# Qixiaomao/video-caption-algorithm

Hardware: AMD Instinct MI355X
Metric: captions/sec + p50 encode+decode latency, 16-frame ViT-B/16 → GPT-2-small, 1/2/4/8 GPU (higher is better)
Workload: dtype bf16

## Files before the change

include/vcap.h:

```cpp
#ifndef VCAP_H_
#define VCAP_H_

#include <stddef.h>
#include <stdint.h>

#ifdef __cplusplus
extern "C" {
#endif

#define VCAP_ABI_VERSION 16

enum { VCAP_DT_F32 = 0, VCAP_DT_BF16 = 1, VCAP_DT_MXFP8 = 2, VCAP_DT_F16 = 3 };
enum { VCAP_E_ARG = -1000, VCAP_E_WORKSPACE = -1001, VCAP_E_UNSUPPORTED = -1002 };

typedef struct vcap_vit_layer {
  const float* ln1_g; const float* ln1_b;
  const void* qkv_w; const float* qkv_b;
  const void* proj_w; const float* proj_b;
  const float* ln2_g; const float* ln2_b;
  const void* fc1_w; const float* fc1_b;
  const void* fc2_w; const float* fc2_b;
  const uint8_t* qkv_ws; const uint8_t* proj_ws; const uint8_t* fc1_ws; const uint8_t* fc2_ws;
} vcap_vit_layer;

// ... 88 lines not shown
                           size_t ws_bytes, void* stream);

size_t vcap_mx_scale_bytes(int rows, int K);
int vcap_vit_attention_mx(const void* qkv, void* out, uint8_t* out_scales, int frames, int tokens, int heads,
                          void* stream);
int vcap_mx_quantize(int in_dtype, const void* x, int64_t ldx, int rows, int K, void* q, uint8_t* scales,
                     void* stream);
int vcap_layernorm_mx(const float* x, int64_t ldx, void* q, uint8_t* scales, const float* gamma, const float* beta,
                      int rows, int dim, float eps, void* stream);
int vcap_gemm_mx(const void* A, const uint8_t* a_scales, const void* W, const uint8_t* w_scales, int out_dtype,
                 void* C, int64_t ldc, uint8_t* c_scales, int M, int N, int K, const float* bias, int act,
                 const float* res, void* stream);
int vcap_vit_pool_temporal(int dtype, const void* feat, void* out, int bsz, int timesteps, int tokens, int channels,
                           int pool_gap, void* stream);
int vcap_prefix_project(const float* emb, int B, int video_dim, const vcap_prefix_desc* pd, float* prefix_out,
                        void* stream);

size_t vcap_rows_packed_bytes(int dtype, int N, int K);
int vcap_rows_pack(int dtype, const void* w, int64_t ldw, int N, int K, void* packed, void* stream);

size_t vcap_vit_workspace_bytes(const vcap_vit_desc* d, int B, int T);
int vcap_vit_encode(const vcap_vit_desc* d, const vcap_prefix_desc* pd, const float* frames, int B, int T,
                    float* enc_out, float* prefix_out, void* workspace, size_t ws_bytes, void* stream);
int vcap_vit_layer_fuses_qkv_attention(const vcap_vit_desc* d, int layer);

size_t vcap_gpt2_workspace_bytes(const vcap_gpt2_desc* d, int B, int S0, int max_new_tokens);
int vcap_gpt2_generate(const vcap_gpt2_desc* d, const vcap_gen_params* gp, const float* prefix, const int* prompt_ids,
                       int prompt_len, int B, int* out_ids, float* logits_out, void* workspace, size_t ws_bytes,
                       void* stream);
typedef struct vcap_sample_params {
  float temperature;
  int top_k;
  double top_p;
  uint64_t seed;
} vcap_sample_params;
int vcap_gpt2_sample(const vcap_gpt2_desc* d, const vcap_gen_params* gp, const vcap_sample_params* sp,
                     const float* prefix, const int* prompt_ids, int prompt_len, int B, int* out_ids,
                     float* logits_out, float* warped_out, const int* force_ids, void* workspace, size_t ws_bytes,
                     void* stream);
void vcap_graph_cache_clear(void);
int vcap_graph_cache_size(void);
int vcap_gpt2_max_rows(void);

int vcap_decode_attention(int dtype, const void* q, const void* k_pool, const void* v_pool, const int* page_table,
                          int maxp, void* out, int M, int heads, int S_new, int past, void* stream);

// ... 156 lines not shown
```

video-caption-algorithm_amd/csrc/gemm256.hip:

```cpp
#include <cstdlib>

#include "vcap_common.h"
#include "vcap_kernels.h"

namespace {

constexpr int TM = 256, TN = 256, ROWB = 128;
constexpr int HALF = 128 * ROWB;
constexpr int BUF = 4 * HALF;
constexpr int LDS_BYTES = 2 * BUF;
constexpr int SBUF = 2048;
constexpr int LDS_BYTES_MX = LDS_BYTES + 4 * SBUF;

VCAP_DEV void glds16(const void* g, char* lds_wave_base) {
  __builtin_amdgcn_global_load_lds((const __attribute__((address_space(1))) void*)g,
                                   (__attribute__((address_space(3))) void*)lds_wave_base, 16, 0, 0);
}

template <typename T, int GS>
VCAP_DEV void half_offsets(uint32_t (&off)[2], long ld, int rows, int base, int X, int wave, int lane) {
  constexpr int E = Frag<T>::kElems;
#pragma unroll
  for (int i = 0; i < 2; ++i) {
    const int lr = (wave * 2 + i) * 8 + (lane >> 3);
// ... 139 lines not shown
          r[i][j] = *reinterpret_cast<const f32x4*>(epi.res + (long)m * epi.ldr + n);
        }
    };
    auto res_store = [&](const f32x4 (&r)[4][2], int qm, int qn) {
#pragma unroll
      for (int i = 0; i < 4; ++i)
#pragma unroll
        for (int j = 0; j < 2; ++j) {
          const int m = m0 + wr * 128 + qm * 64 + i * 16 + fr;
          const int n = n0 + wc * 64 + qn * 32 + j * 16 + fg * 4;
          const f32x4 v = Autocast<TIn>::rnd4(acc[qm][qn][i][j] + bias[qn][j]) + r[i][j];
          if (m < M && n < N) out_store(reinterpret_cast<f32x4*>(C + (long)m * ldc + n), v);
        }
    };
    f32x4 r0[4][2], r1[4][2];
    res_load(r0, 0, 0);
    res_load(r1, 0, 1);
    res_store(r0, 0, 0);
    res_load(r0, 1, 0);
    res_store(r1, 0, 1);
    res_load(r1, 1, 1);
    res_store(r0, 1, 0);
    res_store(r1, 1, 1);
  } else {
#pragma unroll
  for (int qm = 0; qm < 2; ++qm)
#pragma unroll
    for (int qn = 0; qn < 2; ++qn)
#pragma unroll
      for (int j = 0; j < 2; ++j) {
        const int n = n0 + wc * 64 + qn * 32 + j * 16 + fg * 4;
        if (n >= N) continue;
        const f32x4 bias = epi.bias ? *reinterpret_cast<const f32x4*>(epi.bias + n) : (f32x4){0.f, 0.f, 0.f, 0.f};
#pragma unroll
        for (int i = 0; i < 4; ++i) {
          const int m = m0 + wr * 128 + qm * 64 + i * 16 + fr;
          if (m >= M) continue;
          f32x4 v = acc[qm][qn][i][j] + bias;
          if constexpr (!(EPI == 0 && sizeof(TOut) == 2)) v = Autocast<TIn>::rnd4(v);
          long orow = m;
          if constexpr (EPI == 1) {
#pragma unroll
            for (int e = 0; e < 4; ++e) v[e] = gelu_tanh(v[e]);
          } else if constexpr (EPI == 2) {
            v += *reinterpret_cast<const f32x4*>(epi.res + orow * epi.ldr + n);
          } else if constexpr (EPI == 3) {
// ... 258 lines not shown
    if (w > 0 && w < tiles_n && tiles_n % w == 0) e.colgroup = w;
  }
  hipLaunchKernelGGL((vcap_gemm256_kernel<TIn, TOut, EPI>), dim3(tiles), dim3(512), lds, s, (const TIn*)A, lda,
                     (const TIn*)W, ldw, (TOut*)C, ldc, M, N, K, e);
  return hipGetLastError();
}

template <typename TIn, typename TOut>
static hipError_t launch256(const void* A, long lda, const void* W, long ldw, void* C, long ldc, int M, int N, int K,
                            const GemmEpi& epi, hipStream_t s) {
  if constexpr (sizeof(TOut) == 1) {
    return launch256_epi<TIn, TOut, 4>(A, lda, W, ldw, C, ldc, M, N, K, epi, s);
  } else {
    const bool plain_rows = epi.G == 0;
    if (plain_rows && epi.res_mode == 0 && epi.act == 0)
      return launch256_epi<TIn, TOut, 0>(A, lda, W, ldw, C, ldc, M, N, K, epi, s);
    if constexpr (sizeof(TOut) == sizeof(TIn) || sizeof(TOut) == 2) {
      if (plain_rows && epi.res_mode == 0 && epi.act == 1)
        return launch256_epi<TIn, TOut, 1>(A, lda, W, ldw, C, ldc, M, N, K, epi, s);
    }
    if constexpr (sizeof(TOut) == 4) {
      if (plain_rows && epi.res_mode == 1 && epi.act == 0 && epi.res == (const float*)C && epi.ldr == ldc)
        return launch256_epi<TIn, TOut, 2>(A, lda, W, ldw, C, ldc, M, N, K, epi, s);
    }
    return launch256_epi<TIn, TOut, 3>(A, lda, W, ldw, C, ldc, M, N, K, epi, s);
  }
}

bool vcap_gemm256_ok(int in_dt, int out_dt, long lda, long ldw, long ldc, int M, int N, int K, const GemmEpi& epi) {
  if (!vcap_dt_size(in_dt) || !vcap_dt_size(out_dt)) return false;
  const int bk = 128 / (int)vcap_dt_size(in_dt);
  if (K % (2 * bk) != 0 || N % 16 != 0 || M <= 0) return false;
  const int ein = 16 / (int)vcap_dt_size(in_dt);
  if (in_dt == VCAP_DT_MXFP8 && (!epi.a_scale || !epi.w_scale)) return false;
  if (out_dt == VCAP_DT_MXFP8 && (in_dt != VCAP_DT_MXFP8 || N % 128 || ldc % 16 || epi.act != 1 || !epi.bias ||
                                  !epi.c_scale || epi.G || epi.res_mode))
    return false;
  if (lda % ein || ldw % ein) return false;
  if (ldc % 4) return false;
  if (epi.bias && ((uintptr_t)epi.bias & 15)) return false;
  if (epi.res && (((uintptr_t)epi.res & 15) || epi.ldr % 4)) return false;
  (void)out_dt;
  return true;
}

hipError_t vcap_gemm256_dispatch(int in_dt, int out_dt, const void* A, long lda, const void* W, long ldw, void* C,
// ... 20 lines not shown
```

video-caption-algorithm_amd/csrc/runtime_vit.hip:

```cpp
#include "runtime_common.h"

namespace {

struct VitBufs {
  float* x;
  void* xn;
  void* qkv;
  void* attn;
  void* act;
  uint8_t* xn_s;
  uint8_t* act_s;
  float* splitk;
  size_t splitk_bytes;
};

int vit_adt(int dt) { return dt == VCAP_DT_MXFP8 ? VCAP_DT_BF16 : dt; }

VitBufs carve_vit(Carver& c, const vcap_vit_desc* d, int B, int T) {
  const int tokens = (d->image / d->patch) * (d->image / d->patch) + 1;
  const size_t M = (size_t)B * T * tokens;
  const size_t es = esize(d->dtype), ea = esize(vit_adt(d->dtype));
  const size_t npatch = (size_t)B * T * (tokens - 1);
  VitBufs v;
  const size_t en = es > ea ? es : ea;
// ... 24 lines not shown
    return fail(VCAP_E_UNSUPPORTED, "vit dims must be multiples of the GEMM K step");
  if (d->dtype == VCAP_DT_MXFP8) {
    if (d->dim > 1024) return fail(VCAP_E_UNSUPPORTED, "MXFP8 LayerNorm holds rows of <= 1024 in registers");
    if (d->dim % 256 || d->mlp % 256) return fail(VCAP_E_UNSUPPORTED, "MXFP8 dims must be multiples of 256");
  }
  if (d->image % d->patch) return fail(VCAP_E_ARG, "image not divisible by patch");
  const int tokens = (d->image / d->patch) * (d->image / d->patch) + 1;
  if (tokens > 288) return fail(VCAP_E_UNSUPPORTED, "more than 288 tokens");
  if (!vcap_vit_attention_supported(vit_adt(d->dtype), tokens))
    return fail(VCAP_E_UNSUPPORTED, "vit attention serves 33..192 and 225..256 tokens in fp16 only");
  if (!vcap_vit_head_prefix_supported(d->dim, 1)) return fail(VCAP_E_UNSUPPORTED, "vit dim > 1024 (the head holds a row in LDS)");
  if (!vcap_vit_head_prefix_supported(1, d->video_dim)) return fail(VCAP_E_UNSUPPORTED, "video_dim > 1024");
  return 0;
}

bool vit_layer_fused(const vcap_vit_desc* d, const vcap_vit_layer& ly) {
  const bool mx = d->dtype == VCAP_DT_MXFP8;
  const int g = d->image / d->patch;
  return !(mx && ly.qkv_ws) && !(mx && ly.proj_ws) && vcap_vit_qkv_attention_supported(vit_adt(d->dtype), g * g + 1, d->heads);
}

std::string vit_site(const char* name, bool last) { return std::string("vit.") + name + (last ? ".cls" : ""); }

}

extern "C" {

int vcap_vit_attention(int dtype, const void* qkv, void* out, int frames, int tokens, int heads, void* stream) {
  if (!qkv || !out || frames <= 0 || tokens <= 0 || heads <= 0) return fail(VCAP_E_ARG, "vcap_vit_attention: bad arguments");
  if (tokens > 288) return fail(VCAP_E_UNSUPPORTED, "vcap_vit_attention: tokens > 288");
  VCAP_TRY(vcap_vit_attention_dispatch(dtype, qkv, out, frames, tokens, heads, (hipStream_t)stream),
           "vcap_vit_attention");
  return 0;
}

int vcap_vit_qkv_attention_dt(int dtype, const void* xn, const void* wqkv, const float* bqkv, void* out, int frames,
                              int tokens, int heads, int cls_only, void* stream) {
  if (!xn || !wqkv || !bqkv || !out || frames <= 0 || tokens <= 0 || heads <= 0)
    return fail(VCAP_E_ARG, "vcap_vit_qkv_attention: bad arguments");
  if (dtype != VCAP_DT_BF16 && dtype != VCAP_DT_F16)
    return fail(VCAP_E_ARG, "vcap_vit_qkv_attention: dtype must be VCAP_DT_BF16 or VCAP_DT_F16");
  if (!vcap_vit_qkv_attention_supported(dtype, tokens, heads))
    return fail(VCAP_E_UNSUPPORTED, "vcap_vit_qkv_attention: needs 192 < tokens <= 208 (ViT-B/16) or 256 < tokens <= 272 (ViT-L/14) "
                "and heads*64 <= 4096");
  VCAP_TRY(vcap_vit_qkv_attention_dispatch(dtype, xn, wqkv, bqkv, out, frames, tokens, heads, cls_only ? 1 : 0,
                                           (hipStream_t)stream),
// ... 33 lines not shown
                        void* stream) {
  if (!emb || !pd || !prefix_out || !pd->mapper_w || B <= 0) return fail(VCAP_E_ARG, "vcap_prefix_project: bad arguments");
  if (!vcap_vit_head_prefix_supported(1, video_dim)) return fail(VCAP_E_UNSUPPORTED, "video_dim > 1024");
  VCAP_TRY(vcap_vit_head_prefix_dispatch(nullptr, B, 1, 1, 1, nullptr, nullptr, 0.f, nullptr, nullptr, video_dim,
                                         pd->ln_scale, pd->in_weight, pd->mapper_w, pd->mapper_b,
                                         pd->prefix_len * pd->n_embd, nullptr, prefix_out, emb, nullptr,
                                         (hipStream_t)stream),
           "vcap_prefix_project");
  return 0;
}

size_t vcap_vit_workspace_bytes(const vcap_vit_desc* d, int B, int T) {
  return check_vit(d) ? 0 : carved_bytes([&](Carver& c) { carve_vit(c, d, B, T); });
}

int vcap_vit_layer_fuses_qkv_attention(const vcap_vit_desc* d, int layer) {
  if (int rc = check_vit(d)) return rc;
  if (layer < 0 || layer >= d->depth) return fail(VCAP_E_ARG, "vcap_vit_layer_fuses_qkv_attention: layer out of range");
  return vit_layer_fused(d, d->layers[layer]) ? 1 : 0;
}

int vcap_vit_encode(const vcap_vit_desc* d, const vcap_prefix_desc* pd, const float* frames, int B, int T,
                    float* enc_out, float* prefix_out, void* workspace, size_t ws_bytes, void* stream) {
  if (int rc = check_vit(d)) return rc;
  if (!frames || !enc_out || B <= 0 || T <= 0) return fail(VCAP_E_ARG, "vcap_vit_encode: bad arguments");
  if (prefix_out && (!pd || !pd->mapper_w)) return fail(VCAP_E_ARG, "vcap_vit_encode: prefix desc missing");
  if (ws_bytes < vcap_vit_workspace_bytes(d, B, T)) return fail(VCAP_E_WORKSPACE, "vcap_vit_encode: workspace too small");
  hipStream_t s = (hipStream_t)stream;
  Carver c(workspace);
  VitBufs w = carve_vit(c, d, B, T);
  const int dt = d->dtype, D = d->dim, g = d->image / d->patch, P = g * g, N = P + 1, BT = B * T;
  const int adt = vit_adt(dt);
  const bool mx = dt == VCAP_DT_MXFP8;
  const int M = BT * N;
  auto norm = [&](bool mxq, long ldx, const float* gamma, const float* beta, int rows, const char* where) -> int {
    if (mxq)
      VCAP_TRY(vcap_layernorm_mx_dispatch(w.x, ldx, (uint8_t*)w.xn, w.xn_s, rows, gamma, beta, rows, D, d->ln_eps, s),
               where);
    else
      VCAP_TRY(vcap_layernorm_dispatch(adt, w.x, ldx, w.xn, D, gamma, beta, rows, D, d->ln_eps, s), where);
    return 0;
  };
  VCAP_TRY(vcap_patchify_dispatch(adt, frames, w.act, w.x, d->cls, d->pos, BT, d->image, d->patch, d->kpad, N, D, s),
           "patchify");
  GemmEpi pe{d->patch_b, d->pos, D, 0, 2, P, N, 1, 1};
  VCAP_TRY(vcap_gemm_dispatch(adt, VCAP_DT_F32, w.act, d->kpad, d->patch_w, d->kpad, w.x, D, BT * P, D, d->kpad, pe, s),
           "patch_gemm");
  for (int l = 0; l < d->depth; ++l) {
    const vcap_vit_layer& ly = d->layers[l];
    const bool last = l == d->depth - 1;
    const int Mt = last ? BT : M;
    const std::string probe_attn = vit_site("attention", last);
    const bool mq = mx && ly.qkv_ws, mp = mx && ly.proj_ws, m1 = mx && ly.fc1_ws, m2 = mx && ly.fc2_ws;
    const int dq = mq ? VCAP_DT_MXFP8 : adt, dp = mp ? VCAP_DT_MXFP8 : adt;
    const int d1 = m1 ? VCAP_DT_MXFP8 : adt, d2 = m2 ? VCAP_DT_MXFP8 : adt;
    if (int rc = norm(mq, D, ly.ln1_g, ly.ln1_b, M, "norm1")) return rc;
    GemmEpi e1{ly.qkv_b, nullptr, 0, 0, 0, 0, 0, 0, 0, mq ? w.xn_s : nullptr, mq ? ly.qkv_ws : nullptr, nullptr};
    if (vit_layer_fused(d, ly)) {
      ProbeScope ps(probe_attn.c_str(), s, M);
      VCAP_TRY(vcap_vit_qkv_attention_dispatch(adt, w.xn, ly.qkv_w, ly.qkv_b, w.attn, BT, N, d->heads, last, s),
               "qkv_attention");
    } else {
      {
        ProbeScope ps("vit.qkv", s, M);
        VCAP_TRY(vcap_gemm_dispatch(dq, adt, w.xn, D, ly.qkv_w, D, w.qkv, 3 * D, M, 3 * D, D, e1, s), "qkv");
      }
// ... 47 lines not shown
```

video-caption-algorithm_amd/csrc/vcap_kernels.h:

```cpp
#pragma once
#include <hip/hip_runtime.h>

#include <string>

struct GemmEpi {
  const float* bias;
  const float* res;
  long ldr;
  int act;
  int res_mode;
  int G, Gs, goff;
  int roff;
  const uint8_t* a_scale;
  const uint8_t* w_scale;
  uint8_t* c_scale;
  float* splitk_ws;
  size_t splitk_bytes;
  int colgroup;
};

enum { PRO_LN = 0, PRO_DIRECT = 1 };
enum { EPI_QKV = 0, EPI_RESID = 1, EPI_GELU = 2, EPI_LOGITS = 3, EPI_STORE = 4, EPI_LSE = 5, EPI_RELU = 6,
       EPI_QKV_ROWS = 7 };

// ... 69 lines not shown
int vcap_gemm_k_align(int in_dt);
int vcap_gemm_last_splits();
int vcap_stream_cus(hipStream_t s);
int vcap_device_cus();
bool vcap_gemm256_ok(int in_dt, int out_dt, long lda, long ldw, long ldc, int M, int N, int K, const GemmEpi& epi);
hipError_t vcap_gemm256_dispatch(int in_dt, int out_dt, const void* A, long lda, const void* W, long ldw, void* C,
                                 long ldc, int M, int N, int K, const GemmEpi& epi, hipStream_t s);
void vcap_gemm_set_policy(int p);
hipError_t vcap_layernorm_mx_dispatch(const float* x, long ldx, uint8_t* q, uint8_t* scales, int srows,
                                      const float* gamma, const float* beta, int rows, int D, float eps,
                                      hipStream_t s);
hipError_t vcap_mx_quantize_dispatch(int in_dt, const void* x, long ldx, int rows, int K, uint8_t* q,
                                     uint8_t* scales, int srows, hipStream_t s);
hipError_t vcap_layernorm_dispatch(int out_dt, const float* x, long ldx, void* y, long ldy, const float* gamma,
                                   const float* beta, int rows, int D, float eps, hipStream_t s);
bool vcap_vit_attention_supported(int dt, int N);
hipError_t vcap_vit_attention_dispatch(int dt, const void* qkv, void* out, int BT, int N, int H, hipStream_t s,
                                       int cls_only = 0);
bool vcap_vit_qkv_attention_supported(int dt, int N, int H);
hipError_t vcap_vit_qkv_attention_dispatch(int dt, const void* xn, const void* wqkv, const float* bqkv, void* out,
                                           int BT, int N, int H, int cls_only, hipStream_t s);
hipError_t vcap_vit_attention_mx_dispatch(const void* qkv, void* out, uint8_t* oscale, int BT, int N, int H,
                                          hipStream_t s, int cls_only = 0);
hipError_t vcap_patchify_dispatch(int dt, const float* frames, void* patches, float* x, const float* cls,
                                  const float* pos, int BT, int img, int p, int Kp, int N, int D, hipStream_t s);
bool vcap_vit_head_prefix_supported(int D, int VD);
hipError_t vcap_vit_head_prefix_dispatch(const float* x, int B, int T, int N, int D, const float* ng, const float* nb,
                                         float neps, const float* pw, const float* pb, int VD, float ln_scale,
                                         float in_weight, const float* mw, const float* mb, int MO, float* enc_out,
                                         float* prefix, const float* emb_in, float* emb_scratch, hipStream_t s,
                                         int f16_head = 0);
hipError_t vcap_vit_pool_dispatch(int dt, const void* x, void* y, int B, int T, int tokens, int C, int gap,
                                  hipStream_t s);
hipError_t vcap_rows_gemm_dispatch(int dt, int pro, int epi, const RowsGemmArgs& a, int* nblk_out, hipStream_t s);
hipError_t vcap_rows_pack_dispatch(int dt, const void* w, long ldw, int N, int K, void* packed, hipStream_t s);
size_t vcap_rows_packed_size(int dt, int N, int K);
int vcap_logit_blocks(int V, int M);
struct DecodeKeys {
  const int* page_table = nullptr;
  const int* anc = nullptr;
  int anc_ld = 0;
  const uint8_t* kmask = nullptr;
  int mask_ld = 0;
  const int* row_seq = nullptr;
  const int* row_pos = nullptr;
  int pos_add = 0;
  const int* seq_len = nullptr;
// ... 159 lines not shown
```

video-caption-algorithm_amd/csrc/vit_misc.hip:

```cpp
#include "vcap_common.h"
#include "vcap_kernels.h"

template <typename T>
__global__ __launch_bounds__(256) void vcap_patchify_kernel(const float* __restrict__ frames, T* __restrict__ patches,
                                                            float* __restrict__ x, const float* __restrict__ cls,
                                                            const float* __restrict__ pos, int BT, int img, int p,
                                                            int Kp, int N, int D) {
  const int g = img / p, P = g * g;
  const int row = blockIdx.x;
  if (row >= BT * P) {
    const int bt = row - BT * P;
    float* xr = x + (long)bt * N * D;
    for (int d = threadIdx.x; d < D; d += 256) xr[d] = cls[d] + pos[d];
    return;
  }
  const int bt = row / P, pp = row % P;
  const int py = pp / g, px = pp % g;
  const float* f = frames + (long)bt * 3 * img * img;
  T* out = patches + (long)row * Kp;
  const int K = 3 * p * p;
  for (int k = threadIdx.x; k < Kp; k += 256) {
    float v = 0.f;
    if (k < K) {
      const int c = k / (p * p), rem = k % (p * p), i = rem / p, j = rem % p;
      v = f[((long)c * img + (py * p + i)) * img + (px * p + j)];
    }
    out[k] = Num<T>::from_f(v);
  }
}

template <typename T>
__global__ __launch_bounds__(256) void vcap_patchify8_kernel(const float* __restrict__ frames, T* __restrict__ patches,
                                                             int BT, int img, int p, int Kp) {
  const int g = img / p, P = g * g, K = 3 * p * p, cpr = Kp / 8;
  const long i = (long)blockIdx.x * 256 + threadIdx.x;
  if (i >= (long)BT * P * cpr) return;
  const long row = i / cpr;
  const int k = (int)(i % cpr) * 8;
  f32x4 a = {0.f, 0.f, 0.f, 0.f}, b = a;
  if (k < K) {
    const int bt = (int)(row / P), pp = (int)(row % P);
    const int py = pp / g, px = pp % g;
    const int c = k / (p * p), rem = k % (p * p), y = rem / p, x0 = rem % p;
    const float* src = frames + (((long)bt * 3 + c) * img + (py * p + y)) * img + px * p + x0;
    a = *reinterpret_cast<const f32x4*>(src);
    b = *reinterpret_cast<const f32x4*>(src + 4);
  }
  T* dst = patches + row * Kp + k;
  if constexpr (sizeof(T) == 2) {
    *reinterpret_cast<u32x4*>(dst) = (u32x4){Pack2<T>::pack(a.x, a.y), Pack2<T>::pack(a.z, a.w),
                                             Pack2<T>::pack(b.x, b.y), Pack2<T>::pack(b.z, b.w)};
  } else {
    *reinterpret_cast<f32x4*>(dst) = a;
    *reinterpret_cast<f32x4*>(dst + 4) = b;
  }
}

__global__ __launch_bounds__(256) void vcap_cls_rows_kernel(float* __restrict__ x, const float* __restrict__ cls,
                                                            const float* __restrict__ pos, int N, int D) {
  float* xr = x + (long)blockIdx.x * N * D;
  for (int d = threadIdx.x; d < D; d += 256) xr[d] = cls[d] + pos[d];
}

hipError_t vcap_patchify_dispatch(int dt, const float* frames, void* patches, float* x, const float* cls,
                                  const float* pos, int BT, int img, int p, int Kp, int N, int D, hipStream_t s) {
  const int g = img / p;
  if (p % 8 == 0 && Kp % 8 == 0 && img % 4 == 0) {
    const long chunks = (long)BT * g * g * (Kp / 8);
    const dim3 grid((unsigned)((chunks + 255) / 256));
    if (dt == VCAP_DT_BF16)
      hipLaunchKernelGGL((vcap_patchify8_kernel<bf16_t>), grid, dim3(256), 0, s, frames, (bf16_t*)patches, BT, img, p,
                         Kp);
    else if (dt == VCAP_DT_F16)
      hipLaunchKernelGGL((vcap_patchify8_kernel<f16_t>), grid, dim3(256), 0, s, frames, (f16_t*)patches, BT, img, p,
                         Kp);
    else
      hipLaunchKernelGGL((vcap_patchify8_kernel<float>), grid, dim3(256), 0, s, frames, (float*)patches, BT, img, p,
                         Kp);
    hipLaunchKernelGGL(vcap_cls_rows_kernel, dim3(BT), dim3(256), 0, s, x, cls, pos, N, D);
    return hipGetLastError();
  }
  const dim3 grid(BT * g * g + BT), block(256);
  if (dt == VCAP_DT_BF16)
    hipLaunchKernelGGL((vcap_patchify_kernel<bf16_t>), grid, block, 0, s, frames, (bf16_t*)patches, x, cls, pos, BT,
                       img, p, Kp, N, D);
  else if (dt == VCAP_DT_F16)
    hipLaunchKernelGGL((vcap_patchify_kernel<f16_t>), grid, block, 0, s, frames, (f16_t*)patches, x, cls, pos, BT,
                       img, p, Kp, N, D);
// ... 199 lines not shown
```

video-caption-algorithm_amd/vcap/_native.py:

```python
from __future__ import annotations

import ctypes as C
import os
from pathlib import Path

_LIB_PATH = Path(__file__).resolve().parent / "_lib" / "libvcap_hip.so"
_lib = None

DT_F32, DT_BF16, DT_MXFP8, DT_F16 = 0, 1, 2, 3
ABI_VERSION = 16

vp, i32, i64, f32, sz = C.c_void_p, C.c_int, C.c_int64, C.c_float, C.c_size_t
fp = C.POINTER(C.c_float)


E_ARG, E_WORKSPACE, E_UNSUPPORTED = -1000, -1001, -1002


class VcapError(RuntimeError):
    def __init__(self, msg: str, rc: int = 0):
        super().__init__(msg)
        self.rc = rc


class VitLayer(C.Structure):
    _fields_ = [("ln1_g", vp), ("ln1_b", vp), ("qkv_w", vp), ("qkv_b", vp), ("proj_w", vp), ("proj_b", vp),
                ("ln2_g", vp), ("ln2_b", vp), ("fc1_w", vp), ("fc1_b", vp), ("fc2_w", vp), ("fc2_b", vp),
                ("qkv_ws", vp), ("proj_ws", vp), ("fc1_ws", vp), ("fc2_ws", vp)]


class VitDesc(C.Structure):
    _fields_ = [("dtype", i32), ("dim", i32), ("depth", i32), ("heads", i32), ("patch", i32), ("image", i32),
                ("mlp", i32), ("video_dim", i32), ("kpad", i32), ("ln_eps", f32), ("patch_w", vp),
# ... 88 lines not shown
                        i32, vp]),
    "vcap_gemm_splitk": (i32, [i32, vp, i64, vp, i64, vp, i64, i32, i32, i32, vp, i32, i32, vp, sz, C.POINTER(C.c_int),
                               vp]),
    "vcap_layernorm": (i32, [i32, vp, i64, vp, i64, vp, vp, i32, i32, f32, vp]),
    "vcap_vit_attention": (i32, [i32, vp, vp, i32, i32, i32, vp]),
    "vcap_vit_qkv_attention": (i32, [vp, vp, vp, vp, i32, i32, i32, i32, vp]),
    "vcap_vit_qkv_attention_dt": (i32, [i32, vp, vp, vp, vp, i32, i32, i32, i32, vp]),
    "vcap_frames_workspace_bytes": (sz, [i32, i32, i32, i32, i32]),
    "vcap_frames_preprocess": (i32, [vp, i32, i32, i32, i32, i32, fp, fp, vp, vp, vp, sz, vp]),
    "vcap_jpeg_probe": (i32, [vp, sz, C.POINTER(C.c_int), C.POINTER(C.c_int), C.POINTER(C.c_int)]),
    "vcap_jpeg_workspace_bytes": (sz, [vp, sz, i32]),
    "vcap_jpeg_decode_batch": (i32, [C.POINTER(C.c_void_p), C.POINTER(C.c_size_t), i32, vp, vp, sz, vp]),
    "vcap_mx_scale_bytes": (sz, [i32, i32]),
    "vcap_vit_attention_mx": (i32, [vp, vp, vp, i32, i32, i32, vp]),
    "vcap_mx_quantize": (i32, [i32, vp, i64, i32, i32, vp, vp, vp]),
    "vcap_layernorm_mx": (i32, [vp, i64, vp, vp, vp, vp, i32, i32, f32, vp]),
    "vcap_gemm_mx": (i32, [vp, vp, vp, vp, i32, vp, i64, vp, i32, i32, i32, vp, i32, vp, vp]),
    "vcap_vit_pool_temporal": (i32, [i32, vp, vp, i32, i32, i32, i32, i32, vp]),
    "vcap_prefix_project": (i32, [vp, i32, i32, C.POINTER(PrefixDesc), vp, vp]),
    "vcap_rows_packed_bytes": (sz, [i32, i32, i32]),
    "vcap_rows_pack": (i32, [i32, vp, i64, i32, i32, vp, vp]),
    "vcap_vit_workspace_bytes": (sz, [C.POINTER(VitDesc), i32, i32]),
    "vcap_vit_encode": (i32, [C.POINTER(VitDesc), C.POINTER(PrefixDesc), vp, i32, i32, vp, vp, vp, sz, vp]),
    "vcap_vit_layer_fuses_qkv_attention": (i32, [C.POINTER(VitDesc), i32]),
    "vcap_gpt2_workspace_bytes": (sz, [C.POINTER(GPT2Desc), i32, i32, i32]),
    "vcap_gpt2_generate": (i32, [C.POINTER(GPT2Desc), C.POINTER(GenParams), vp, C.POINTER(C.c_int), i32, i32, vp,
                                 vp, vp, sz, vp]),
    "vcap_gpt2_sample": (i32, [C.POINTER(GPT2Desc), C.POINTER(GenParams), C.POINTER(SampleParams), vp,
                               C.POINTER(C.c_int), i32, i32, vp, vp, vp, vp, vp, sz, vp]),
    "vcap_graph_cache_clear": (None, []),
    "vcap_graph_cache_size": (i32, []),
    "vcap_gpt2_max_rows": (i32, []),
    "vcap_gpt2_beam_search_workspace_bytes": (sz, [C.POINTER(GPT2Desc), i32, i32, i32, i32]),
    "vcap_gpt2_beam_search": (i32, [C.POINTER(GPT2Desc), C.POINTER(BeamParams), vp, C.POINTER(C.c_int), i32, i32,
                                    vp, vp, vp, sz, vp]),
    "vcap_decode_attention": (i32, [i32, vp, vp, vp, vp, i32, vp, i32, i32, i32, i32, vp]),
    "vcap_gpt2_beam_workspace_bytes": (sz, [C.POINTER(GPT2Desc), i32, i32, i32]),
    "vcap_gpt2_prefill": (i32, [C.POINTER(GPT2Desc), vp, C.POINTER(C.c_int), i32, i32, i32, i32, vp, vp, sz, vp]),
    "vcap_gpt2_step": (i32, [C.POINTER(GPT2Desc), vp, i32, i32, i32, i32, vp, vp, sz, vp]),
    "vcap_gpt2_reorder": (i32, [C.POINTER(GPT2Desc), vp, i32, i32, i32, i32, vp, sz, vp]),
    "vcap_gpt2_forward_embeds": (i32, [C.POINTER(GPT2Desc), vp, i32, i32, i32, i32, i32, vp, vp, sz, vp]),
    "vcap_gpt2_score_workspace_bytes": (sz, [C.POINTER(GPT2Desc), i32, i32]),
    "vcap_gpt2_score": (i32, [C.POINTER(GPT2Desc), vp, i32, i32, vp, vp, vp, vp, vp, vp, sz, vp]),
    "vcap_gpt2_score_backward_workspace_bytes": (sz, [C.POINTER(GPT2Desc), C.POINTER(GPT2GradDesc), i32, i32]),
    "vcap_gpt2_score_backward": (i32, [C.POINTER(GPT2Desc), C.POINTER(GPT2GradDesc), vp, i32, i32, vp, vp, vp, vp, vp,
                                       vp, vp, sz, vp]),
# ... 64 lines not shown
```

video-caption-algorithm_amd/vcap/model.py:

```python
from __future__ import annotations

import ctypes as C
from dataclasses import dataclass
from typing import Dict, List, Optional, Sequence, Tuple

import numpy as np
import torch

from . import _native as N
from .configs import VIDEO_DIM, GPT2Arch, ViTArch

_DTYPES = {"bf16": (N.DT_BF16, torch.bfloat16), "fp32": (N.DT_F32, torch.float32)}
_VIT_DTYPES = dict(_DTYPES, fp8=(N.DT_MXFP8, torch.bfloat16), fp16=(N.DT_F16, torch.float16))


def _dtype(mode: str):
    if mode not in _DTYPES:
        raise ValueError(f"precision must be one of {sorted(_DTYPES)}, got {mode!r}")
    return _DTYPES[mode]


def _stream(device) -> int:
    return torch.cuda.current_stream(device).cuda_stream


class _Workspace:
    def __init__(self, device):
# ... 75 lines not shown
                if name in self.mx_gemms:
                    lt[name + "_w"], lt[name + "_ws"] = wmx(b + key)
                else:
                    lt[name + "_w"] = wt(b + key)
            for k, v in lt.items():
                keep(v)
                setattr(self.layers[i], k, v.data_ptr())
        self.desc = N.VitDesc(dtype=self.dt, dim=arch.dim, depth=arch.depth, heads=arch.heads, patch=arch.patch,
                              image=arch.image, mlp=arch.mlp, video_dim=video_dim, kpad=self.kpad,
                              ln_eps=arch.ln_eps, patch_w=self.patch_w.data_ptr(), patch_b=t["patch_b"].data_ptr(),
                              cls=t["cls"].data_ptr(), pos=t["pos"].data_ptr(), norm_g=t["norm_g"].data_ptr(),
                              norm_b=t["norm_b"].data_ptr(), proj_w=t["proj_w"].data_ptr(),
                              proj_b=t["proj_b"].data_ptr(), layers=self.layers)
        self.ws = _Workspace(dev)

    def workspace_bytes(self, B: int, T: int) -> int:
        return int(N.lib().vcap_vit_workspace_bytes(C.byref(self.desc), B, T))

    def fuses_qkv_attention(self, layer: int = 0) -> bool:
        rc = int(N.lib().vcap_vit_layer_fuses_qkv_attention(C.byref(self.desc), int(layer)))
        N.check(min(rc, 0), "vcap_vit_layer_fuses_qkv_attention")
        return rc == 1

    def encode(self, video: torch.Tensor, prefix: Optional["HipPrefix"] = None,
               out_prefix: Optional[torch.Tensor] = None):
        if video.dim() == 4:
            video = video.unsqueeze(1)
        if video.dim() != 5:
            raise ValueError(f"expect [B,T,3,H,W], got {tuple(video.shape)}")
        B, T, Cc, H, W = video.shape
        a = self.arch
        if Cc != 3 or H != a.image or W != a.image:
            raise ValueError(f"expect frames of 3x{a.image}x{a.image}, got {tuple(video.shape)}")
        if video.device != self.device and not (video.is_cuda and self.device.type == "cuda"):
            raise ValueError("video must be on the encoder's device")
        video = video.to(torch.float32).contiguous()
        enc = torch.empty(B, self.video_dim, dtype=torch.float32, device=video.device)
        pre = None
        pd = None
        if prefix is not None:
            shape = (B, prefix.prefix_len, prefix.n_embd)
            if out_prefix is not None:
                if tuple(out_prefix.shape) != shape or out_prefix.dtype != torch.float32 or not out_prefix.is_contiguous():
                    raise ValueError(f"out_prefix must be contiguous f32 {shape}")
                pre = out_prefix
            else:
                pre = torch.empty(*shape, dtype=torch.float32, device=video.device)
            pd = C.byref(prefix.desc)
        nbytes = self.workspace_bytes(B, T)
        ws = self.ws.get(nbytes)
        N.check(N.lib().vcap_vit_encode(C.byref(self.desc), pd, video.data_ptr(), B, T, enc.data_ptr(),
                                        N.ptr(pre), ws.data_ptr(), ws.numel(), _stream(video.device)),
                "vcap_vit_encode")
        return enc, pre


class HipPrefix:

    def __init__(self, sd: Dict[str, np.ndarray], n_embd: int, prefix_len: int = 4, ln_scale: float = 0.6,
                 in_weight: float = 0.4, device="cuda"):
        dev = torch.device(device)
        self.prefix_len, self.n_embd = prefix_len, n_embd
        self.mapper_w = torch.from_numpy(np.ascontiguousarray(sd["decoder.mapper.0.weight"], np.float32)).to(dev)
        self.mapper_b = torch.from_numpy(np.ascontiguousarray(sd["decoder.mapper.0.bias"], np.float32)).to(dev)
        if self.mapper_w.shape[0] != prefix_len * n_embd:
            raise ValueError(f"mapper out {self.mapper_w.shape[0]} != prefix_len*n_embd {prefix_len * n_embd}")
        self.set_scales(ln_scale, in_weight)

    def set_scales(self, ln_scale: Optional[float], in_weight: Optional[float]) -> None:
        self.ln_scale = float(ln_scale) if ln_scale is not None else 0.0
        self.in_weight = float(in_weight) if in_weight is not None else 0.0
        self.desc = N.PrefixDesc(ln_scale=self.ln_scale, in_weight=self.in_weight, prefix_len=self.prefix_len,
                                 n_embd=self.n_embd, mapper_w=self.mapper_w.data_ptr(),
                                 mapper_b=self.mapper_b.data_ptr())

    def project(self, emb: torch.Tensor) -> torch.Tensor:
# ... 433 lines not shown
```

video-caption-algorithm_amd/vcap/pipeline.py:

```python
from __future__ import annotations

from typing import List, Optional, Sequence, Union

import atexit
import ctypes as C

import torch

from . import _native as N
from . import trace
from .model import GenConfig, HipGPT2Decoder, HipPrefix, HipViTEncoder, _Workspace


_STREAM_SETS: dict = {}


def _device_index(device) -> int:
    d = torch.device(device)
    return d.index if d.index is not None else torch.cuda.current_device()


def _stream_set(device, reserve_cus: int, confine_decode, lanes: int):
    device = torch.device("cuda", _device_index(device))
    ndec = reserve_cus if confine_decode is True else int(confine_decode or 0)
# ... 40 lines not shown
def _release_at_exit() -> None:
    try:
        if _STREAM_SETS and torch.cuda.is_initialized():
            release_streams()
    except Exception:
        pass


atexit.register(_release_at_exit)


class CaptionPipeline:
    def __init__(self, encoder: HipViTEncoder, prefix: HipPrefix, decoder: HipGPT2Decoder, cfg: GenConfig,
                 batch: int, prompt_ids: Sequence[int], device, depth: int = 2, gather=None,
                 reserve_cus: int = 0, dec_lanes: int = 1, confine_decode: Union[bool, int] = False, dec_group: int = 1,
                 enc_group: int = 1):
        self.enc, self.pre, self.dec, self.cfg = encoder, prefix, decoder, cfg
        self.prompt_ids = list(prompt_ids)
        self.device = torch.device("cuda", _device_index(device))
        if dec_lanes < 1 or dec_group < 1 or enc_group < 1:
            raise ValueError("dec_lanes, dec_group and enc_group must be >= 1")
        if dec_group % enc_group:
            raise ValueError(f"enc_group ({enc_group}) must divide dec_group ({dec_group})")
        self.lanes = int(dec_lanes)
        self.group = int(dec_group)
        self.egroup = int(enc_group)
        self._stage = None
        self._staged = 0
        self._pending_mid: List[torch.cuda.Event] = []
        self.batch = int(batch)
        depth = max(int(depth), self.lanes + 1)
        self.depth = depth
        self.s_enc, self.s_decs = _stream_set(self.device, int(reserve_cus),
                                              confine_decode if isinstance(confine_decode, bool) else int(confine_decode),
                                              self.lanes)
        self.s_dec = self.s_decs[0]
        cur = torch.cuda.current_stream(self.device)
        for st in [self.s_enc] + self.s_decs:
            st.wait_stream(cur)
        self.dec_ws = [decoder.ws] + [_Workspace(self.device) for _ in range(self.lanes - 1)]
        E = decoder.arch.n_embd
        G = self.group
        self.group_prefix = [torch.empty(G * batch, prefix.prefix_len, E, device=self.device) for _ in range(depth)]
        self.group_ids = [torch.empty(G * batch, cfg.max_new_tokens, dtype=torch.int32, device=self.device)
                          for _ in range(depth)]
        self.enc_done = [torch.cuda.Event() for _ in range(depth)]
        self.dec_done: List[Optional[torch.cuda.Event]] = [None] * depth
        self.gather = gather
        self.outputs: List[Optional[torch.Tensor]] = [None] * (depth * G)
        self._pending_end: List[torch.cuda.Event] = []
        self.k = 0

    @property
    def prefix_bufs(self) -> List[torch.Tensor]:
        B = self.batch
        return [gp[j * B:(j + 1) * B] for gp in self.group_prefix for j in range(self.group)]

    def submit(self, video: torch.Tensor, t_start: Optional[torch.cuda.Event] = None,
               t_mid: Optional[torch.cuda.Event] = None, t_end: Optional[torch.cuda.Event] = None) -> int:
        G, B, E = self.group, self.batch, self.egroup
        g, j = divmod(self.k, G)
        slot = g % self.depth
        with torch.cuda.stream(self.s_enc):
            if j == 0 and self.dec_done[slot] is not None:
                self.s_enc.wait_event(self.dec_done[slot])
            if t_start is not None:
                t_start.record()
            if t_mid is not None:
                self._pending_mid.append(t_mid)
            if E == 1:
                self._encode(video, slot, j, 1)
            else:
                if self._stage is None or self._stage.shape[1:] != video.shape[1:] or self._stage.dtype != video.dtype:
                    self._stage = torch.empty((E * B,) + tuple(video.shape[1:]), dtype=video.dtype, device=self.device)
                self._stage[self._staged * B:(self._staged + 1) * B].copy_(video)
                self._staged += 1
                if self._staged == E:
                    self._encode(self._stage, slot, j - E + 1, E)
        if t_end is not None:
            self._pending_end.append(t_end)
        self.k += 1
        self.last_slot = slot * G + j
        if j == G - 1:
            self._decode_group(g)
        return self.last_slot

    def _encode(self, video: torch.Tensor, slot: int, j0: int, n: int) -> None:
        B = self.batch
        with trace.range(trace.VIT):
            self.enc.encode(video[:n * B], self.pre, out_prefix=self.group_prefix[slot][j0 * B:(j0 + n) * B])
        for ev in self._pending_mid:
            ev.record()
        self._pending_mid = []
        self.enc_done[slot].record()
        self._staged = 0

    def flush(self) -> None:
        if self.k % self.group:
            g = self.k // self.group
            if self._staged:
                with torch.cuda.stream(self.s_enc):
                    j = self.k % self.group
                    self._encode(self._stage, g % self.depth, j - self._staged, self._staged)
            self.k = (g + 1) * self.group
            self._decode_group(g)

    def _decode_group(self, g: int) -> None:
        G, B = self.group, self.batch
        slot, lane = g % self.depth, g % self.lanes
        s_dec = self.s_decs[lane]
        with torch.cuda.stream(s_dec):
            s_dec.wait_event(self.enc_done[slot])
            with trace.range(trace.DECODE):
                self.dec.generate_ids(self.group_prefix[slot], self.prompt_ids, self.cfg, out=self.group_ids[slot],
                                      workspace=self.dec_ws[lane])
            out = self.group_ids[slot]
            if self.gather is not None:
                out = self.gather(out, g * G)
            for i in range(G):
                self.outputs[slot * G + i] = out[i * B:(i + 1) * B]
            for ev in self._pending_end:
                ev.record()
            self._pending_end = []
            ev = torch.cuda.Event()
            ev.record()
            self.dec_done[slot] = ev
# ... 16 lines not shown
```

Baseline: 1301.

## Read encode-group frame batches in place instead of staging into one buffer

Encoder grouping no longer copies each submitted video batch into a contiguous staging tensor. A list of up to four frame pointers is passed down to the patchify kernel, which picks the source batch for each frame index. A new GEMM epilogue variant (EPI 5) handles grouped row remapping with a positional residual using the paired load/store schedule. Together these remove a device-to-device copy per submitted batch and give the patch-embedding epilogue a specialised path. In exchange, the held caller tensors must stay alive until the encode runs.

Result: no change. 1312, median of 6 (+0.9%).

```diff
diff --git a/include/vcap.h b/include/vcap.h
--- a/include/vcap.h
+++ b/include/vcap.h
@@ -134,6 +134,10 @@
 size_t vcap_vit_workspace_bytes(const vcap_vit_desc* d, int B, int T);
 int vcap_vit_encode(const vcap_vit_desc* d, const vcap_prefix_desc* pd, const float* frames, int B, int T,
                     float* enc_out, float* prefix_out, void* workspace, size_t ws_bytes, void* stream);
+#define VCAP_MAX_FRAME_BATCHES 4
+int vcap_vit_encode_batches(const vcap_vit_desc* d, const vcap_prefix_desc* pd, const float* const* frames, int nb,
+                            int B, int T, float* enc_out, float* prefix_out, void* workspace, size_t ws_bytes,
+                            void* stream);
 int vcap_vit_layer_fuses_qkv_attention(const vcap_vit_desc* d, int layer);
 
 size_t vcap_gpt2_workspace_bytes(const vcap_gpt2_desc* d, int B, int S0, int max_new_tokens);
diff --git a/video-caption-algorithm_amd/csrc/gemm256.hip b/video-caption-algorithm_amd/csrc/gemm256.hip
--- a/video-caption-algorithm_amd/csrc/gemm256.hip
+++ b/video-caption-algorithm_amd/csrc/gemm256.hip
@@ -185,6 +185,59 @@
     res_load(r1, 1, 1);
     res_store(r0, 1, 0);
     res_store(r1, 1, 1);
+  } else if constexpr (EPI == 5) {
+    f32x4 bias[2][2];
+#pragma unroll
+    for (int qn = 0; qn < 2; ++qn)
+#pragma unroll
+      for (int j = 0; j < 2; ++j) {
+        const int n = min(n0 + wc * 64 + qn * 32 + j * 16 + fg * 4, N - 4);
+        bias[qn][j] = epi.bias ? *reinterpret_cast<const f32x4*>(epi.bias + n) : (f32x4){0.f, 0.f, 0.f, 0.f};
+      }
+    int mq[2][4], mr[2][4];
+    auto rows = [&](int qm) {
+#pragma unroll
+      for (int i = 0; i < 4; ++i) {
+        const int m = min(m0 + wr * 128 + qm * 64 + i * 16 + fr, M - 1);
+        mq[qm][i] = m / epi.G;
+        mr[qm][i] = m - mq[qm][i] * epi.G;
+      }
+    };
+    auto pos_load = [&](f32x4 (&r)[4][2], int qm, int qn) {
+#pragma unroll
+      for (int i = 0; i < 4; ++i) {
+        const float* row = epi.res + (long)(mr[qm][i] + epi.roff) * epi.ldr;
+#pragma unroll
+        for (int j = 0; j < 2; ++j) {
+          const int n = min(n0 + wc * 64 + qn * 32 + j * 16 + fg * 4, N - 4);
+          r[i][j] = *reinterpret_cast<const f32x4*>(row + n);
+        }
+      }
+    };
+    auto pos_store = [&](const f32x4 (&r)[4][2], int qm, int qn) {
+#pragma unroll
+      for (int i = 0; i < 4; ++i) {
+        const int m = m0 + wr * 128 + qm * 64 + i * 16 + fr;
+        TOut* row = C + ((long)mq[qm][i] * epi.Gs + epi.goff + mr[qm][i]) * ldc;
+#pragma unroll
+        for (int j = 0; j < 2; ++j) {
+          const int n = n0 + wc * 64 + qn * 32 + j * 16 + fg * 4;
+          const f32x4 v = Autocast<TIn>::rnd4(acc[qm][qn][i][j] + bias[qn][j]) + r[i][j];
+          if (m < M && n < N) out_store(reinterpret_cast<f32x4*>(row + n), v);
+        }
+      }
+    };
+    f32x4 r0[4][2], r1[4][2];
+    rows(0);
+    pos_load(r0, 0, 0);
+    pos_load(r1, 0, 1);
+    pos_store(r0, 0, 0);
+    rows(1);
+    pos_load(r0, 1, 0);
+    pos_store(r1, 0, 1);
+    pos_load(r1, 1, 1);
+    pos_store(r0, 1, 0);
+    pos_store(r1, 1, 1);
   } else {
 #pragma unroll
   for (int qm = 0; qm < 2; ++qm)
@@ -489,6 +542,8 @@
     if constexpr (sizeof(TOut) == 4) {
       if (plain_rows && epi.res_mode == 1 && epi.act == 0 && epi.res == (const float*)C && epi.ldr == ldc)
         return launch256_epi<TIn, TOut, 2>(A, lda, W, ldw, C, ldc, M, N, K, epi, s);
+      if (epi.G > 0 && epi.res_mode == 2 && epi.act == 0 && epi.res)
+        return launch256_epi<TIn, TOut, 5>(A, lda, W, ldw, C, ldc, M, N, K, epi, s);
     }
     return launch256_epi<TIn, TOut, 3>(A, lda, W, ldw, C, ldc, M, N, K, epi, s);
   }
diff --git a/video-caption-algorithm_amd/csrc/runtime_vit.hip b/video-caption-algorithm_amd/csrc/runtime_vit.hip
--- a/video-caption-algorithm_amd/csrc/runtime_vit.hip
+++ b/video-caption-algorithm_amd/csrc/runtime_vit.hip
@@ -70,6 +70,9 @@
 
 std::string vit_site(const char* name, bool last) { return std::string("vit.") + name + (last ? ".cls" : ""); }
 
+int vit_encode(const char* who, const vcap_vit_desc* d, const vcap_prefix_desc* pd, const float* const* frames, int nb,
+               int Bb, int T, float* enc_out, float* prefix_out, void* workspace, size_t ws_bytes, void* stream);
+
 }
 
 extern "C" {
@@ -149,10 +152,35 @@
 
 int vcap_vit_encode(const vcap_vit_desc* d, const vcap_prefix_desc* pd, const float* frames, int B, int T,
                     float* enc_out, float* prefix_out, void* workspace, size_t ws_bytes, void* stream) {
+  return vit_encode("vcap_vit_encode", d, pd, &frames, 1, B, T, enc_out, prefix_out, workspace, ws_bytes, stream);
+}
+
+int vcap_vit_encode_batches(const vcap_vit_desc* d, const vcap_prefix_desc* pd, const float* const* frames, int nb,
+                            int B, int T, float* enc_out, float* prefix_out, void* workspace, size_t ws_bytes,
+                            void* stream) {
+  return vit_encode("vcap_vit_encode_batches", d, pd, frames, nb, B, T, enc_out, prefix_out, workspace, ws_bytes,
+                    stream);
+}
+
+}
+
+namespace {
+
+int vit_encode(const char* who, const vcap_vit_desc* d, const vcap_prefix_desc* pd, const float* const* frames, int nb,
+               int Bb, int T, float* enc_out, float* prefix_out, void* workspace, size_t ws_bytes, void* stream) {
+  const std::string me(who);
   if (int rc = check_vit(d)) return rc;
-  if (!frames || !enc_out || B <= 0 || T <= 0) return fail(VCAP_E_ARG, "vcap_vit_encode: bad arguments");
-  if (prefix_out && (!pd || !pd->mapper_w)) return fail(VCAP_E_ARG, "vcap_vit_encode: prefix desc missing");
-  if (ws_bytes < vcap_vit_workspace_bytes(d, B, T)) return fail(VCAP_E_WORKSPACE, "vcap_vit_encode: workspace too small");
+  if (!frames || !enc_out || nb <= 0 || Bb <= 0 || T <= 0) return fail(VCAP_E_ARG, me + ": bad arguments");
+  if (nb > VCAP_MAX_FRAME_BATCHES) return fail(VCAP_E_ARG, me + ": more than VCAP_MAX_FRAME_BATCHES batches");
+  FrameSrc fs;
+  for (int i = 0; i < 4; ++i) {
+    fs.batch[i] = frames[i < nb ? i : 0];
+    if (!fs.batch[i]) return fail(VCAP_E_ARG, me + ": bad arguments");
+  }
+  fs.per = Bb * T;
+  const int B = nb * Bb;
+  if (prefix_out && (!pd || !pd->mapper_w)) return fail(VCAP_E_ARG, me + ": prefix desc missing");
+  if (ws_bytes < vcap_vit_workspace_bytes(d, B, T)) return fail(VCAP_E_WORKSPACE, me + ": workspace too small");
   hipStream_t s = (hipStream_t)stream;
   Carver c(workspace);
   VitBufs w = carve_vit(c, d, B, T);
@@ -168,7 +196,7 @@
       VCAP_TRY(vcap_layernorm_dispatch(adt, w.x, ldx, w.xn, D, gamma, beta, rows, D, d->ln_eps, s), where);
     return 0;
   };
-  VCAP_TRY(vcap_patchify_dispatch(adt, frames, w.act, w.x, d->cls, d->pos, BT, d->image, d->patch, d->kpad, N, D, s),
+  VCAP_TRY(vcap_patchify_dispatch(adt, fs, w.act, w.x, d->cls, d->pos, BT, d->image, d->patch, d->kpad, N, D, s),
            "patchify");
   GemmEpi pe{d->patch_b, d->pos, D, 0, 2, P, N, 1, 1};
   VCAP_TRY(vcap_gemm_dispatch(adt, VCAP_DT_F32, w.act, d->kpad, d->patch_w, d->kpad, w.x, D, BT * P, D, d->kpad, pe, s),
diff --git a/video-caption-algorithm_amd/csrc/vcap_kernels.h b/video-caption-algorithm_amd/csrc/vcap_kernels.h
--- a/video-caption-algorithm_amd/csrc/vcap_kernels.h
+++ b/video-caption-algorithm_amd/csrc/vcap_kernels.h
@@ -115,7 +115,11 @@
                                            int BT, int N, int H, int cls_only, hipStream_t s);
 hipError_t vcap_vit_attention_mx_dispatch(const void* qkv, void* out, uint8_t* oscale, int BT, int N, int H,
                                           hipStream_t s, int cls_only = 0);
-hipError_t vcap_patchify_dispatch(int dt, const float* frames, void* patches, float* x, const float* cls,
+struct FrameSrc {
+  const float* batch[4];
+  int per;
+};
+hipError_t vcap_patchify_dispatch(int dt, const FrameSrc& frames, void* patches, float* x, const float* cls,
                                   const float* pos, int BT, int img, int p, int Kp, int N, int D, hipStream_t s);
 bool vcap_vit_head_prefix_supported(int D, int VD);
 hipError_t vcap_vit_head_prefix_dispatch(const float* x, int B, int T, int N, int D, const float* ng, const float* nb,
diff --git a/video-caption-algorithm_amd/csrc/vit_misc.hip b/video-caption-algorithm_amd/csrc/vit_misc.hip
--- a/video-caption-algorithm_amd/csrc/vit_misc.hip
+++ b/video-caption-algorithm_amd/csrc/vit_misc.hip
@@ -1,8 +1,14 @@
 #include "vcap_common.h"
 #include "vcap_kernels.h"
 
+VCAP_DEV const float* frame_of(const FrameSrc& fs, int bt, int img) {
+  const int q = bt / fs.per, r = bt - q * fs.per;
+  const float* b = q == 0 ? fs.batch[0] : (q == 1 ? fs.batch[1] : (q == 2 ? fs.batch[2] : fs.batch[3]));
+  return b + (long)r * 3 * img * img;
+}
+
 template <typename T>
-__global__ __launch_bounds__(256) void vcap_patchify_kernel(const float* __restrict__ frames, T* __restrict__ patches,
+__global__ __launch_bounds__(256) void vcap_patchify_kernel(const FrameSrc frames, T* __restrict__ patches,
                                                             float* __restrict__ x, const float* __restrict__ cls,
                                                             const float* __restrict__ pos, int BT, int img, int p,
                                                             int Kp, int N, int D) {
@@ -16,7 +22,7 @@
   }
   const int bt = row / P, pp = row % P;
   const int py = pp / g, px = pp % g;
-  const float* f = frames + (long)bt * 3 * img * img;
+  const float* f = frame_of(frames, bt, img);
   T* out = patches + (long)row * Kp;
   const int K = 3 * p * p;
   for (int k = threadIdx.x; k < Kp; k += 256) {
@@ -30,8 +36,8 @@
 }
 
 template <typename T>
-__global__ __launch_bounds__(256) void vcap_patchify8_kernel(const float* __restrict__ frames, T* __restrict__ patches,
-                                                             int BT, int img, int p, int Kp) {
+__global__ __launch_bounds__(256) void vcap_patchify8_kernel(const FrameSrc frames, T* __restrict__ patches, int BT,
+                                                             int img, int p, int Kp) {
   const int g = img / p, P = g * g, K = 3 * p * p, cpr = Kp / 8;
   const long i = (long)blockIdx.x * 256 + threadIdx.x;
   if (i >= (long)BT * P * cpr) return;
@@ -42,7 +48,7 @@
     const int bt = (int)(row / P), pp = (int)(row % P);
     const int py = pp / g, px = pp % g;
     const int c = k / (p * p), rem = k % (p * p), y = rem / p, x0 = rem % p;
-    const float* src = frames + (((long)bt * 3 + c) * img + (py * p + y)) * img + px * p + x0;
+    const float* src = frame_of(frames, bt, img) + ((long)c * img + (py * p + y)) * img + px * p + x0;
     a = *reinterpret_cast<const f32x4*>(src);
     b = *reinterpret_cast<const f32x4*>(src + 4);
   }
@@ -62,8 +68,9 @@
   for (int d = threadIdx.x; d < D; d += 256) xr[d] = cls[d] + pos[d];
 }
 
-hipError_t vcap_patchify_dispatch(int dt, const float* frames, void* patches, float* x, const float* cls,
+hipError_t vcap_patchify_dispatch(int dt, const FrameSrc& frames, void* patches, float* x, const float* cls,
                                   const float* pos, int BT, int img, int p, int Kp, int N, int D, hipStream_t s) {
+  if (frames.per <= 0 || BT > 4 * (long)frames.per) return hipErrorInvalidValue;
   const int g = img / p;
   if (p % 8 == 0 && Kp % 8 == 0 && img % 4 == 0) {
     const long chunks = (long)BT * g * g * (Kp / 8);
diff --git a/video-caption-algorithm_amd/vcap/_native.py b/video-caption-algorithm_amd/vcap/_native.py
--- a/video-caption-algorithm_amd/vcap/_native.py
+++ b/video-caption-algorithm_amd/vcap/_native.py
@@ -9,6 +9,7 @@
 
 DT_F32, DT_BF16, DT_MXFP8, DT_F16 = 0, 1, 2, 3
 ABI_VERSION = 16
+MAX_FRAME_BATCHES = 4
 
 vp, i32, i64, f32, sz = C.c_void_p, C.c_int, C.c_int64, C.c_float, C.c_size_t
 fp = C.POINTER(C.c_float)
@@ -143,6 +144,8 @@
     "vcap_rows_pack": (i32, [i32, vp, i64, i32, i32, vp, vp]),
     "vcap_vit_workspace_bytes": (sz, [C.POINTER(VitDesc), i32, i32]),
     "vcap_vit_encode": (i32, [C.POINTER(VitDesc), C.POINTER(PrefixDesc), vp, i32, i32, vp, vp, vp, sz, vp]),
+    "vcap_vit_encode_batches": (i32, [C.POINTER(VitDesc), C.POINTER(PrefixDesc), C.POINTER(C.c_void_p), i32, i32, i32,
+                                      vp, vp, vp, sz, vp]),
     "vcap_vit_layer_fuses_qkv_attention": (i32, [C.POINTER(VitDesc), i32]),
     "vcap_gpt2_workspace_bytes": (sz, [C.POINTER(GPT2Desc), i32, i32, i32]),
     "vcap_gpt2_generate": (i32, [C.POINTER(GPT2Desc), C.POINTER(GenParams), vp, C.POINTER(C.c_int), i32, i32, vp,
diff --git a/video-caption-algorithm_amd/vcap/model.py b/video-caption-algorithm_amd/vcap/model.py
--- a/video-caption-algorithm_amd/vcap/model.py
+++ b/video-caption-algorithm_amd/vcap/model.py
@@ -2,7 +2,7 @@
 
 import ctypes as C
 from dataclasses import dataclass
-from typing import Dict, List, Optional, Sequence, Tuple
+from typing import Dict, List, Optional, Sequence, Tuple, Union
 
 import numpy as np
 import torch
@@ -124,19 +124,30 @@
         N.check(min(rc, 0), "vcap_vit_layer_fuses_qkv_attention")
         return rc == 1
 
-    def encode(self, video: torch.Tensor, prefix: Optional["HipPrefix"] = None,
-               out_prefix: Optional[torch.Tensor] = None):
+    def _frames(self, video: torch.Tensor) -> torch.Tensor:
         if video.dim() == 4:
             video = video.unsqueeze(1)
         if video.dim() != 5:
             raise ValueError(f"expect [B,T,3,H,W], got {tuple(video.shape)}")
-        B, T, Cc, H, W = video.shape
         a = self.arch
-        if Cc != 3 or H != a.image or W != a.image:
+        if video.shape[2] != 3 or video.shape[3] != a.image or video.shape[4] != a.image:
             raise ValueError(f"expect frames of 3x{a.image}x{a.image}, got {tuple(video.shape)}")
         if video.device != self.device and not (video.is_cuda and self.device.type == "cuda"):
             raise ValueError("video must be on the encoder's device")
-        video = video.to(torch.float32).contiguous()
+        return video.to(torch.float32).contiguous()
+
+    def encode(self, video: Union[torch.Tensor, Sequence[torch.Tensor]], prefix: Optional["HipPrefix"] = None,
+               out_prefix: Optional[torch.Tensor] = None):
+        batches = [self._frames(v) for v in (video if isinstance(video, (list, tuple)) else [video])]
+        if not 1 <= len(batches) <= N.MAX_FRAME_BATCHES:
+            raise ValueError(f"expect 1..{N.MAX_FRAME_BATCHES} frame tensors, got {len(batches)}")
+        video = batches[0]
+        for v in batches[1:]:
+            if v.shape != video.shape or v.device != video.device:
+                raise ValueError(f"frame tensors of one encode must share shape and device, got {tuple(video.shape)} "
+                                 f"and {tuple(v.shape)}")
+        nb, (Bb, T) = len(batches), video.shape[:2]
+        B = nb * Bb
         enc = torch.empty(B, self.video_dim, dtype=torch.float32, device=video.device)
         pre = None
         pd = None
@@ -151,9 +162,10 @@
             pd = C.byref(prefix.desc)
         nbytes = self.workspace_bytes(B, T)
         ws = self.ws.get(nbytes)
-        N.check(N.lib().vcap_vit_encode(C.byref(self.desc), pd, video.data_ptr(), B, T, enc.data_ptr(),
-                                        N.ptr(pre), ws.data_ptr(), ws.numel(), _stream(video.device)),
-                "vcap_vit_encode")
+        ptrs = (C.c_void_p * nb)(*[v.data_ptr() for v in batches])
+        N.check(N.lib().vcap_vit_encode_batches(C.byref(self.desc), pd, ptrs, nb, Bb, T, enc.data_ptr(), N.ptr(pre),
+                                                ws.data_ptr(), ws.numel(), _stream(video.device)),
+                "vcap_vit_encode_batches")
         return enc, pre
 
 
diff --git a/video-caption-algorithm_amd/vcap/pipeline.py b/video-caption-algorithm_amd/vcap/pipeline.py
--- a/video-caption-algorithm_amd/vcap/pipeline.py
+++ b/video-caption-algorithm_amd/vcap/pipeline.py
@@ -86,11 +86,12 @@
             raise ValueError("dec_lanes, dec_group and enc_group must be >= 1")
         if dec_group % enc_group:
             raise ValueError(f"enc_group ({enc_group}) must divide dec_group ({dec_group})")
+        if enc_group > N.MAX_FRAME_BATCHES:
+            raise ValueError(f"enc_group ({enc_group}) > {N.MAX_FRAME_BATCHES}, the batches one encode reads in place")
         self.lanes = int(dec_lanes)
         self.group = int(dec_group)
         self.egroup = int(enc_group)
-        self._stage = None
-        self._staged = 0
+        self._held: List[torch.Tensor] = []
         self._pending_mid: List[torch.cuda.Event] = []
         self.batch = int(batch)
         depth = max(int(depth), self.lanes + 1)
@@ -132,15 +133,9 @@
                 t_start.record()
             if t_mid is not None:
                 self._pending_mid.append(t_mid)
-            if E == 1:
-                self._encode(video, slot, j, 1)
-            else:
-                if self._stage is None or self._stage.shape[1:] != video.shape[1:] or self._stage.dtype != video.dtype:
-                    self._stage = torch.empty((E * B,) + tuple(video.shape[1:]), dtype=video.dtype, device=self.device)
-                self._stage[self._staged * B:(self._staged + 1) * B].copy_(video)
-                self._staged += 1
-                if self._staged == E:
-                    self._encode(self._stage, slot, j - E + 1, E)
+            self._held.append(video)
+            if len(self._held) == E:
+                self._encode(slot, j - E + 1)
         if t_end is not None:
             self._pending_end.append(t_end)
         self.k += 1
@@ -149,23 +144,23 @@
             self._decode_group(g)
         return self.last_slot
 
-    def _encode(self, video: torch.Tensor, slot: int, j0: int, n: int) -> None:
-        B = self.batch
+    def _encode(self, slot: int, j0: int) -> None:
+        held, self._held = self._held, []
+        B, n = self.batch, len(held)
         with trace.range(trace.VIT):
-            self.enc.encode(video[:n * B], self.pre, out_prefix=self.group_prefix[slot][j0 * B:(j0 + n) * B])
+            self.enc.encode([v[:B] for v in held], self.pre, out_prefix=self.group_prefix[slot][j0 * B:(j0 + n) * B])
         for ev in self._pending_mid:
             ev.record()
         self._pending_mid = []
         self.enc_done[slot].record()
-        self._staged = 0
 
     def flush(self) -> None:
         if self.k % self.group:
             g = self.k // self.group
-            if self._staged:
+            if self._held:
                 with torch.cuda.stream(self.s_enc):
                     j = self.k % self.group
-                    self._encode(self._stage, g % self.depth, j - self._staged, self._staged)
+                    self._encode(g % self.depth, j - len(self._held))
             self.k = (g + 1) * self.group
             self._decode_group(g)
 
```
